# h3jia/bayesfast

Hardware: AMD Instinct MI355X
Metric: leapfrog steps/sec (all chains), 4096 chains x 64-d quadratic surrogate (higher is better)
Workload: dtype f64

## Files before the change

### bayesfast_amd/csrc/bfhip_api.hip

```cpp
#include <cmath>
#include <cstdarg>
#include <cstdio>
#include <cstdlib>
#include <cstring>
#include <vector>
#include "bfhip_common.h"
#include "bfhip_pack.h"

static thread_local char g_err[512] = "";

int bf_set_error(int code, const char *fmt, ...) {
    va_list ap;
    va_start(ap, fmt);
    vsnprintf(g_err, sizeof(g_err), fmt, ap);
    va_end(ap);
    return code;
}

static int env_int(const char *name, int dflt) { const char *e = getenv(name); return e ? atoi(e) : dflt; }
BfTune &bf_tune() {
    static BfTune t = [] {
        BfTune u;
        memset(&u, 0, sizeof(u));
        const char *nk = getenv("BFHIP_NUTS_KERNEL");
        u.no_group = env_int("BFHIP_NO_GROUP", (nk && (!strcmp(nk, "sliced") || !strcmp(nk, "pipe"))) ? 1 : 0);
        u.no_pipe = env_int("BFHIP_NO_PIPE", (nk && !strcmp(nk, "sliced")) ? 1 : 0);
        u.no_plain = env_int("BFHIP_NO_PLAIN", 0);
        u.no_quad = env_int("BFHIP_NO_QUAD", 0);
        u.wave_cpg = env_int("BFHIP_WAVE_CPG", 0);
        u.tail_relaunch = env_int("BFHIP_TAIL_RELAUNCH", 1);
        u.tail_stop = env_int("BFHIP_TAIL_STOP", 4);
        u.tail_q = env_int("BFHIP_TAIL_Q", 3);
        u.tail_max = env_int("BFHIP_TAIL_MAX", 4);
        u.lone = env_int("BFHIP_LONE", 1);
        u.lone_form = env_int("BFHIP_LONE_FORM", -1);
        u.pld_waves = env_int("BFHIP_PLD_WAVES", 0);
        u.cubic_form = env_int("BFHIP_CUBIC_FORM", 0);
        u.cubic_loops = env_int("BFHIP_CUBIC_LOOPS", 0);
        u.gram_one_wave = env_int("BFHIP_GRAM_ONE_WAVE", 0);
        u.chol_one_panel = env_int("BFHIP_CHOL_ONE_PANEL", 0);
        u.no_vel_ahead = env_int("BFHIP_NO_VEL_AHEAD", 0);
        u.tnuts_wpb = env_int("BFHIP_TNUTS_WPB", 0);
        u.tnuts_generic = env_int("BFHIP_TNUTS_GENERIC", 0);
        u.no_bound_proof = env_int("BFHIP_NO_BOUND_PROOF", 0);
        u.no_proof_weights = env_int("BFHIP_NO_PROOF_WEIGHTS", 0);
        u.pld_no_compress = env_int("BFHIP_PLD_NO_COMPRESS", 0);
        u.pld_stream = env_int("BFHIP_PLD_STREAM", 0);
        u.pld_no_cl = env_int("BFHIP_PLD_NO_CL", 0);
        u.no_decay_shared = env_int("BFHIP_NO_DECAY_SHARED", 0);
        u.polar_tiles = env_int("BFHIP_POLAR_TILES", 0);
        u.no_group_pld = env_int("BFHIP_NO_GROUP_PLD", 0);
        return u;
    }();
    return t;
}
static int *tune_field(const char *key) {
    BfTune &t = bf_tune();
    struct { const char *k; int *p; } tab[] = {
        {"no_group", &t.no_group}, {"no_pipe", &t.no_pipe}, {"no_plain", &t.no_plain}, {"no_quad", &t.no_quad}, {"wave_cpg", &t.wave_cpg},
        {"tail_relaunch", &t.tail_relaunch}, {"tail_stop", &t.tail_stop}, {"tail_q", &t.tail_q}, {"tail_max", &t.tail_max}, {"lone", &t.lone}, {"lone_form", &t.lone_form},
        {"pld_waves", &t.pld_waves}, {"cubic_form", &t.cubic_form}, {"cubic_loops", &t.cubic_loops}, {"gram_one_wave", &t.gram_one_wave}, {"chol_one_panel", &t.chol_one_panel}, {"no_vel_ahead", &t.no_vel_ahead}, {"tnuts_wpb", &t.tnuts_wpb}, {"tnuts_generic", &t.tnuts_generic}, {"no_bound_proof", &t.no_bound_proof},
        {"no_proof_weights", &t.no_proof_weights}, {"pld_no_compress", &t.pld_no_compress}, {"pld_stream", &t.pld_stream}, {"pld_no_cl", &t.pld_no_cl}, {"no_decay_shared", &t.no_decay_shared}, {"polar_tiles", &t.polar_tiles}, {"no_group_pld", &t.no_group_pld}};
    for (auto &e : tab)
        if (key && !strcmp(key, e.k)) return e.p;
    return NULL;
}
extern "C" int bfhip_debug_set(const char *key, long long value) {
    int *f = tune_field(key);
    if (!f) return bf_set_error(BFHIP_ERR_ARG, "bfhip_debug_set: unknown switch '%s'", key ? key : "(null)");
    *f = (int)value;
    return 0;
}
extern "C" long long bfhip_debug_get(const char *key) {
    const int *f = tune_field(key);
    return f ? *f : 0;
}
extern "C" int bfhip_debug_buffer(const char *key, void *device_ptr) {
    BfTune &t = bf_tune();
    unsigned long long *p = (unsigned long long *)device_ptr;
    if (key && !strcmp(key, "stamps")) t.stamps = p;
    else if (key && !strcmp(key, "stamps_lone")) t.stamps_lone = p;
    else if (key && !strcmp(key, "gstamps")) t.gstamps = p;
    else if (key && !strcmp(key, "group_counters")) t.group_counters = p;
    else return bf_set_error(BFHIP_ERR_ARG, "bfhip_debug_buffer: unknown buffer '%s'", key ? key : "(null)");
    return 0;
}
extern "C" const char *bfhip_debug_last_kernel(void) { return bf_tune().last_kernel; }

extern "C" int bfhip_version(void) { return 108; }
extern "C" const char *bfhip_last_error(void) { return g_err; }

extern "C" int bfhip_ctx_create(bfhip_ctx **out, int device, void *stream) {
    if (!out) return bf_set_error(BFHIP_ERR_ARG, "bfhip_ctx_create: out is NULL");
    int n_dev = 0;
    BF_HIP_CHECK(hipGetDeviceCount(&n_dev));
    if (device < 0 || device >= n_dev) return bf_set_error(BFHIP_ERR_ARG, "bfhip_ctx_create: device %d of %d", device, n_dev);
    BF_HIP_CHECK(hipSetDevice(device));
    hipDeviceProp_t prop;
    BF_HIP_CHECK(hipGetDeviceProperties(&prop, device));
    if (strncmp(prop.gcnArchName, "gfx950", 6) != 0)
        return bf_set_error(BFHIP_ERR_UNSUPPORTED, "bfhip is built for gfx950 only, found %s", prop.gcnArchName);
    bfhip_ctx *c = (bfhip_ctx *)calloc(1, sizeof(bfhip_ctx));
    c->device = device;
    c->stream = (hipStream_t)stream;
    c->n_cu = prop.multiProcessorCount;
    *out = c;
    return 0;
}

extern "C" void bfhip_ctx_destroy(bfhip_ctx *ctx) {
    if (!ctx) return;
    if (ctx->model_buf) (void)hipFree(ctx->model_buf);
    if (ctx->scratch) (void)hipFree(ctx->scratch);
    if (ctx->cubic_buf) (void)hipFree(ctx->cubic_buf);
    if (ctx->pm_buf) (void)hipFree(ctx->pm_buf);
    if (ctx->pld_buf) (void)hipFree(ctx->pld_buf);
    if (ctx->tail_buf) (void)hipFree(ctx->tail_buf);
    if (ctx->flow) (void)hipFree(ctx->flow);
    if (ctx->hess_work) (void)hipFree(ctx->hess_work);
    free(ctx);
}

extern "C" int bfhip_ctx_set_stream(bfhip_ctx *ctx, void *stream) {
    if (!ctx) return bf_set_error(BFHIP_ERR_ARG, "ctx is NULL");
    ctx->stream = (hipStream_t)stream;
    return 0;
}

extern "C" int bfhip_ctx_synchronize(bfhip_ctx *ctx) {
    if (!ctx) return bf_set_error(BFHIP_ERR_ARG, "ctx is NULL");
    BF_HIP_CHECK(hipStreamSynchronize(ctx->stream));
    return 0;
}

extern "C" int bfhip_density_upload(bfhip_ctx *ctx, const bfhip_density_desc *ds) {
    BfDeviceGuard dev_guard(ctx);
    if (!ctx || !ds) return bf_set_error(BFHIP_ERR_ARG, "bfhip_density_upload: NULL argument");
    const int d = ds->d;
    if (d < 1 || d > BFHIP_MAX_DIM) return bf_set_error(BFHIP_ERR_ARG, "bfhip_density_upload: d = %d out of [1, %d]", d, BFHIP_MAX_DIM);
    if (ds->use_bound && (!ds->mu || !ds->hess || !(ds->alpha > 0.)))
        return bf_set_error(BFHIP_ERR_ARG, "use_bound needs mu, hess and alpha > 0");
    if (ds->use_decay && (!ds->decay_mu || !ds->decay_hess))
        return bf_set_error(BFHIP_ERR_ARG, "use_decay needs decay_mu and decay_hess");
    if ((ds->su_lo == NULL) != (ds->su_diff == NULL)) return bf_set_error(BFHIP_ERR_ARG, "su_lo and su_diff go together");
    std::vector<double> h;
    const int DP = bf_pack_density(ds, h);
    const size_t MAT = (size_t)DP * DP, n_dbl = h.size();
    BF_HIP_CHECK(hipSetDevice(ctx->device));
    const size_t bytes = n_dbl * sizeof(double);
    if (int rc = bf_grow(ctx, &ctx->model_buf, &ctx->model_bytes, bytes)) return rc;
    BF_HIP_CHECK(hipStreamSynchronize(ctx->stream));
    BF_HIP_CHECK(hipMemcpy(ctx->model_buf, h.data(), bytes, hipMemcpyHostToDevice));
    DevModel &m = ctx->model;
    memset(&m, 0, sizeof(m));
    m.d = d;
    m.DP = DP;
    m.has_transform = ds->ranges != NULL;
    m.has_su = ds->su_lo != NULL;
    m.has_quad = ds->quad != NULL;
    m.use_bound = ds->use_bound != 0;
    m.use_decay = ds->use_decay != 0;
    m.decay_shared = ds->use_bound && ds->use_decay && memcmp(ds->decay_hess, ds->hess, (size_t)d * d * sizeof(double)) == 0 &&
                     memcmp(ds->decay_mu, ds->mu, (size_t)d * sizeof(double)) == 0;
    const double *base = (const double *)ctx->model_buf;
    m.pd = base;
    m.Sf = base + (size_t)PD_N * DP;
    m.Hf = m.Sf + MAT;
    m.Hdf = m.Hf + MAT;
    if (m.decay_shared) m.Hdf = m.Hf;
    m.c0 = ds->c0;
    m.alpha = ds->alpha;
    m.lam_max = ds->use_bound ? bf_bound_lam_max_weighted(ds->hess, ds->d, h.data() + (size_t)PD_HD * DP) : 0.;
    m.lam_max_d = ds->use_decay ? bf_bound_lam_max_weighted(ds->decay_hess, ds->d, h.data() + (size_t)PD_HDD * DP) : 0.;
    m.f_mu = ds->f_mu;
// ... 128 lines not shown
```

### bayesfast_amd/csrc/bfhip_common.h

```cpp
#pragma once
#include <hip/hip_runtime.h>
#include <stdint.h>
#include "../../include/bfhip.h"
#include "bfhip_model.h"
#include "bfhip_tune.h"

__device__ inline double bf_shfl_xor(double v, int mask) { return __shfl_xor(v, mask, 64); }

__device__ inline double bf_logaddexp(double x, double y) {
    if (x == y) return x + 0.6931471805599453094;
    double tmp = x - y;
    if (tmp > 0) return x + log1p(exp(-tmp));
    if (tmp <= 0) return y + log1p(exp(tmp));
    return tmp;
}

__device__ inline uint64_t bf_order_key(double v) {
    if (v != v) return ~0ull;
    if (v == 0.) v = 0.;
    const uint64_t b = (uint64_t)__double_as_longlong(v);
    return (b >> 63) ? ~b : (b | 0x8000000000000000ull);
}

#define BF_HIP_CHECK(expr)                                                                 \
// ... 13 lines not shown
    size_t model_bytes;
    void *cubic_buf;
    size_t cubic_bytes;
    void *pm_buf;
    size_t pm_bytes;
    int has_pm;
    void *pld_buf;
    size_t pld_bytes;
    struct PolyDev {
        int d, DP, m, use_bound, has_quad;
        const double *Sf;
        const double *lin;
        const double *c0;
        const double *f_mu;
        const double *mu;
        const double *Hf;
        double alpha;
        int n2, n3;
        const int *mask2, *pos2, *mask3, *pos3;
        const double *A2, *A2t, *T3t;
    } pm;
    int *tail_buf;
    size_t tail_bytes;
    void *scratch;
    size_t scratch_bytes;
    int n_cu;
    void *flow;
    size_t flow_bytes;
    void *hess_work;
    size_t hess_work_bytes;
};

struct BfDeviceGuard {
    int prev = -1;
    explicit BfDeviceGuard(const bfhip_ctx *ctx) {
        if (ctx && hipGetDevice(&prev) == hipSuccess && prev != ctx->device) (void)hipSetDevice(ctx->device);
        else prev = -1;
    }
    ~BfDeviceGuard() { if (prev >= 0) (void)hipSetDevice(prev); }
};

#define BF_LDS_MAX ((size_t)160 * 1024)

template <typename K>
static inline int bf_set_lds(K kern, size_t bytes) {
    if (bytes > 64 * 1024)
// ... 23 lines not shown
```

### bayesfast_amd/csrc/bfhip_lone.h

```cpp

#pragma push_macro("exp")
#pragma push_macro("log")
#pragma push_macro("sqrt")
#pragma push_macro("sincospi")
#undef exp
#undef log
#undef sqrt
#undef sincospi
__device__ inline double ln_opq(double x) { asm("" : "+v"(x)); return x; }
#define LN_EXPV(x) ln_opq(exp(ln_opq(x)))
#define LN_LOGV(x) ln_opq(log(ln_opq(x)))
#define LN_SQRTV(x) ln_opq(sqrt(ln_opq(x)))
#define LN_EXP(x) rfl(LN_EXPV(x))
#define LN_LOG(x) rfl(LN_LOGV(x))
#define LN_SQRT(x) rfl(LN_SQRTV(x))

enum { LN_CONT = 0, LN_NEW = 1, LN_DONE = 2 };
enum { LF_NONE = 0, LF_LEAF = 1, LF_INIT = 2 };
enum { LV_CMD = 0, LV_CLOSE, LV_EO, LV_EVAL, LV_DIR, LV_INIT, LV_N = 8 };

template <int W, int DEC>
struct LoneGeo {
    using PG = PipeGeo<W, DEC>;
    static constexpr int DP = 16 * W, NS = 4 * W, NMAT = PG::NMAT, KS = PG::KS, KPJ = PG::KPJ;
// ... 711 lines not shown
                    dir_use = bf_pipe_dir(bf_xoshiro_next(t));
                }
            }
            if (lane == 0) {
                VI[LV_CMD] = LN_CONT; VI[LV_CLOSE] = close; VI[LV_EO] = eo; VI[LV_EVAL] = ev; VI[LV_DIR] = dir_use;
            }
            fly = ev ? LF_LEAF : LF_NONE;
        }
        LTRACE(1, 3);
#ifdef BF_LTRACE
        ltrip += 1;
#endif
    }
#undef KBAR

#ifdef BF_LTRACE
    if (a.stamps && blockIdx.x == 0)
        for (int i = lane; i < BF_LTRACE * 32; i += 64) a.stamps[i] = LTRC[i];
#endif
    if (err == 2 && lane_ok) q = LF[lane];
    store_vec(BFHIP_VEC_Q, q);
    if (lane == 0) {
        for (int k = 0; k < 4; ++k) a.rng[(size_t)chain * 4 + k] = rs[k];
        scp[BFHIP_SC_LOG_STEP] = log_step;
        scp[BFHIP_SC_LOG_BAR] = log_bar;
        scp[BFHIP_SC_HBAR] = hbar;
        scp[BFHIP_SC_COUNT] = count;
        scp[BFHIP_SC_I_ITER] = (double)i_iter;
        scp[BFHIP_SC_ERROR] = (double)err;
        if (a.n_leapfrog && nlf) atomicAdd(a.n_leapfrog, nlf);
    }
}
#undef LN_EXP
#undef LN_LOG
#undef LN_SQRT
#undef LN_EXPV
#undef LN_LOGV
#undef LN_SQRTV
#pragma pop_macro("exp")
#pragma pop_macro("log")
#pragma pop_macro("sqrt")
#pragma pop_macro("sincospi")
```

### bayesfast_amd/csrc/bfhip_nuts_pipe.h

```cpp


enum { SL_PROPG = SL_STACK + 4 * BFHIP_MAX_TREEDEPTH, SL_PG = SL_PROPG + 1, SL_PIPE_N = SL_PG + BFHIP_MAX_TREEDEPTH };

template <int W, int DEC = 0>
struct PipeGeo {
    static constexpr int NMAT = DEC == 1 ? 3 : 2;
    static constexpr int KS = DEC == 1 ? (W == 2 ? 2 : 1) : ((W == 2 || W == 4) ? 2 : 1);
    static constexpr int KPJ = (4 * W) / KS, NJOB = NMAT * W * KS, NTL = 12;
    static constexpr int MPS = KPJ > 8 ? 2 : 1;
    static_assert(NJOB <= 16 && KPJ <= 8 * MPS, "one job per wave, eight MFMA sites");
    static constexpr size_t lds_doubles() {
        using G = SamplerGeo<W>;
        return (size_t)NMAT * G::NS * G::XS + (size_t)16 * BFHIP_MAX_TREEDEPTH * LS_N + 4 + (size_t)16 * CS_N +
               (size_t)16 * NTL * G::DP + (size_t)NMAT * KS * 16 * G::GS;
    }
};

template <int QUAD> struct PipeAcc { typedef d4_t type; };
template <> struct PipeAcc<1> { typedef double type; };
template <> struct PipeAcc<2> { typedef d2_t type; };
__device__ inline d4_t bf_pipe_mfma(double a_, double b_, d4_t c_) { return __builtin_amdgcn_mfma_f64_16x16x4f64(a_, b_, c_, 0, 0, 0); }
__device__ inline double bf_pipe_mfma(double a_, double b_, double c_) { return __builtin_amdgcn_mfma_f64_4x4x4f64(a_, b_, c_, 0, 0, 0); }

__device__ inline double bf_pipe_u01(uint64_t x) {
// ... 12 lines not shown
    constexpr int DP = G::DP, NS = G::NS, XS = G::XS, GS = G::GS;
    constexpr int KS_P = PG::KS, KPJ_P = PG::KPJ, NJOB_P = PG::NJOB, NTL = PG::NTL, NMAT = PG::NMAT, MPS = PG::MPS;
    constexpr int MAXL = BFHIP_MAX_TREEDEPTH;
    static_assert(DP <= 64, "one dimension per lane");
    extern __shared__ __attribute__((aligned(16))) double lds[];
    double *XB = lds;
    double *LS = XB + NMAT * NS * XS;
    int *alive = (int *)(LS + 16 * MAXL * LS_N);
    double *CS = LS + 16 * MAXL * LS_N + 4;
    double *TB = CS + 16 * CS_N;
    double *GB = TB + 16 * NTL * DP;

    const int tid = threadIdx.x, lane = tid & 63;
    const int w = __builtin_amdgcn_readfirstlane(tid >> 6);
    int cpg = a.cpg > 0 ? a.cpg : 16;
    int chain = blockIdx.x * cpg + w;
    bool real = w < cpg && chain < a.n_chain;
    if (a.tail_list) {
        const int cnt = rfl(a.tail_count[0]);
        cpg = cnt <= a.n_cu ? 1 : (cnt <= 2 * a.n_cu ? 2 : 4);
        const int idx = blockIdx.x * cpg + w;
        real = w < cpg && idx < cnt;
        chain = real ? rfl(a.tail_list[idx]) : 0;
    }
    const int d = m.d;
    const bool lane_ok = lane < DP;

    double afr[KPJ_P];
    {
        const int slot_m = w / (W * KS_P), rem = w % (W * KS_P), t = rem / KS_P, kp = rem % KS_P;
        const double *Af = (slot_m == 0 ? m.Sf : (slot_m == 1 ? m.Hf : m.Hdf)) + (t * NS + kp * KPJ_P) * 64 + lane;
#pragma unroll
        for (int s = 0; s < KPJ_P; ++s) afr[s] = (w < NJOB_P) ? Af[s * 64] : 0.;
    }
    if (tid < 8) alive[tid] = 0;
    const double c_lin = lane_ok ? m.pd[PD_LIN * DP + lane] : 0.;
    const double c_mu = lane_ok ? m.pd[PD_MU * DP + lane] : 0.;
    const double c_dmu = (DEC == 1 && lane_ok) ? m.pd[PD_DMU * DP + lane] : 0.;
    const double c_smu = lane_ok ? m.pd[PD_SMU * DP + lane] : 0.;
    const int c_kind = (TR && lane_ok) ? (int)m.pd[PD_KIND * DP + lane] : 0;
    const double c_lo = (TR && lane_ok) ? m.pd[PD_LO * DP + lane] : 0., c_rg = (TR && lane_ok) ? m.pd[PD_RG * DP + lane] : 1.;
    double xs = 0., jac = 1., gj = 0., logdet_l = 0.;

    double q = 0., p = 0., g = 0., var = 1.;
    double TLp = 0., TPs = 0., TPq = 0.;
    double TRp = 0.;
// ... 44 lines not shown
        double sn, cs;
        sincospi(2. * u2, &sn, &cs);
        const double z = (lane & 1) ? rad * sn : rad * cs;
        p = (lane < d) ? (1. / sqrt(var)) * z : 0.;
        g = 0.;
    };
    if (real) {
        for (int k = 0; k < 4; ++k) rs[k] = rfl((uint64_t)a.rng[(size_t)chain * 4 + k]);
        cs_set(CS_LOG_STEP, rfl(scp[BFHIP_SC_LOG_STEP]));
        cs_set(CS_LOG_BAR, rfl(scp[BFHIP_SC_LOG_BAR]));
        cs_set(CS_HBAR, rfl(scp[BFHIP_SC_HBAR]));
        cs_set(CS_SMU, rfl(scp[BFHIP_SC_MU]));
        cs_set(CS_COUNT, rfl(scp[BFHIP_SC_COUNT]));
        cs_set(CS_STEP_NOW, uexp(rfl(scp[BFHIP_SC_LOG_STEP])));
        cs_set(CS_STEP_BAR, uexp(rfl(scp[BFHIP_SC_LOG_BAR])));
        i_iter = rfl((int)scp[BFHIP_SC_I_ITER]);
        err = rfl((int)scp[BFHIP_SC_ERROR]);
        q = load_vec(BFHIP_VEC_Q, 0.);
        var = load_vec(BFHIP_VEC_VAR, 1.);
        if (i_iter < a.iter_end && err == 0) {
            mode = M_INIT;
            draw_momentum();
        } else if (a.tail_done && lane == 0) {
            atomicAdd(a.tail_done, 1);
        }
    }
    __syncthreads();
    if (lane == 0 && mode == M_DONE) atomicAdd(&alive[6], 1);

#ifdef BF_TRACE
    __shared__ unsigned long long TRC[BF_TRACE * 16];
    for (int i = threadIdx.x; i < BF_TRACE * 16; i += 1024) TRC[i] = 0;
    int trip_no = 0;
#endif
    auto init_tree = [&](double E0, double logp0) {
        if (!(fabs(E0) <= 1.7976931348623157e308)) {
            err = 1;
        } else {
            start_energy = E0;
            stv(SL_LEFT_Q, q); stv(SL_LEFT_P, p); stv(SL_LEFT_G, g);
            stv(SL_RIGHT_Q, q); stv(SL_RIGHT_P, p); stv(SL_RIGHT_G, g);
            stv(SL_PROP_Q, q); stv(SL_PSUM, p);
            stv(SL_PROPG, g);
            cs_set(CS_PROP_E, E0);
            cs_set(CS_PROP_LOGP, logp0);
            cs_set(CS_TREE_W, 1.);
            w_off = 0.;
// ... 73 lines not shown
                    prev_upd = n_samples;
                    if (a.cfg.doubling) adapt_window *= 2.;
                }
                n_samples += 1.;
                store_vec(BFHIP_VEC_FG_MEAN, fm);
                store_vec(BFHIP_VEC_FG_RAW, fr);
                store_vec(BFHIP_VEC_BG_MEAN, bm);
                store_vec(BFHIP_VEC_BG_RAW, br);
                if (lane == 0) {
                    scp[BFHIP_SC_FG_N] = fg_n;
                    scp[BFHIP_SC_BG_N] = bg_n;
                    scp[BFHIP_SC_N_SAMPLES] = n_samples;
                    scp[BFHIP_SC_PREV_UPDATE] = prev_upd;
                    scp[BFHIP_SC_ADAPT_WINDOW] = adapt_window;
                }
            }
            i_iter += 1;
            TRACE(12);
            bool go_on = i_iter < a.iter_end && err == 0;
            if (go_on && a.tail_stop > 0 && a.iter_end - i_iter >= 8) {
                const int i_iter0 = rfl((int)scp[BFHIP_SC_I_ITER]);
                if (4 * (a.iter_end - i_iter) >= a.iter_end - i_iter0 && 16 - rfl(alive[6]) <= a.tail_stop) {
                    const int dg = rfl(__hip_atomic_load(a.tail_done, __ATOMIC_RELAXED, __HIP_MEMORY_SCOPE_AGENT));
                    if (4 * dg >= a.tail_q * a.n_chain) go_on = false;
                }
            }
            if (go_on) {
                mode = M_INIT;
                draw_momentum();
            } else {
                mode = M_DONE;
                if (lane == 0) {
                    atomicAdd(&alive[6], 1);
                    if (a.tail_done && (i_iter >= a.iter_end || err != 0)) atomicAdd(a.tail_done, 1);
                }
            }
        }
    };

    auto gb_read = [&](int slot_m) -> double {
        const double *gp = GB + ((slot_m * KS_P) * 16 + w) * GS + lane;
        double r = gp[0];
        if (KS_P > 1) r += gp[16 * GS];
        return r;
    };

    for (int trip = 0;; ++trip) {
#ifdef BF_TRACE
        trip_no = trip;
#endif
        TRACE(0);
        bool evaluating = false, turn = false;
        int eo2 = 0;
        if (mode == M_INIT) {
            evaluating = true;
        } else if (mode == M_LEAF) {
            evaluating = true;
// ... 383 lines not shown
                } else if constexpr (DEC == 2) {
                    r_a[0] = pc.get(2); r_a[1] = pc.get(3);
                } else {
                    r_a[0] = xm * gmu; r_a[1] = xm * sv;
                    wave_sum_n<2>(r_a);
                }
                const BfOob o = bf_oob_scalars(m.alpha, m.inv_alpha, m.f_mu, m.f_poly_mu, beta, r_a[0], r_a[1]);
                f = o.f;
                gn = bf_oob_grad(o, gmu, sv, hv);
                kin_ready = false;
            }
            finish(f, gn, kin_ready, r_kin, logdet, r_bd2, dgr);
        }
    }

#ifdef BF_TRACE
    if (a.stamps && w == 0 && blockIdx.x == 0)
        for (int i = lane; i < BF_TRACE * 16; i += 64) a.stamps[i] = TRC[i];
#endif
    if (real) {
        store_vec(BFHIP_VEC_Q, q);
        if (lane == 0) {
            for (int k = 0; k < 4; ++k) a.rng[(size_t)chain * 4 + k] = rs[k];
            scp[BFHIP_SC_LOG_STEP] = cs_get(CS_LOG_STEP);
            scp[BFHIP_SC_LOG_BAR] = cs_get(CS_LOG_BAR);
            scp[BFHIP_SC_HBAR] = cs_get(CS_HBAR);
            scp[BFHIP_SC_COUNT] = cs_get(CS_COUNT);
            scp[BFHIP_SC_I_ITER] = (double)i_iter;
            scp[BFHIP_SC_ERROR] = (double)err;
            if (a.n_leapfrog && nlf) atomicAdd(a.n_leapfrog, nlf);
        }
    }
}
```

### bayesfast_amd/csrc/bfhip_sampler.hip

```cpp
#include <type_traits>
#include <cstring>
#include <cstdio>
#include <cstdlib>
#include "bfhip_eval.h"
#include "bfhip_metric.h"
#include "bfhip_pld.h"
#include "bfhip_oob.h"

__device__ __attribute__((noinline)) static double bf_exp_ni(double x) { return exp(x); }
__device__ __attribute__((noinline)) static double bf_log_ni(double x) { return log(x); }
__device__ __attribute__((noinline)) static double bf_sqrt_ni(double x) { return sqrt(x); }
__device__ __attribute__((noinline)) static void bf_sincospi_ni(double x, double *s, double *c) { sincospi(x, s, c); }
#define exp(x) bf_exp_ni(x)
#define log(x) bf_log_ni(x)
#define sqrt(x) bf_sqrt_ni(x)
#define sincospi(x, s, c) bf_sincospi_ni(x, s, c)
#define uexp(x) rfl(bf_exp_ni(x))
#define ulog(x) rfl(bf_log_ni(x))
#define usqrt(x) rfl(bf_sqrt_ni(x))

#include "bfhip_sampler_defs.h"

#include "bfhip_wave.h"

// ... 1637 lines not shown
    args.cub_lds = sampler_cubic_lds(ctx->model, FS == 1) ? 1 : 0;
    args.cub_loops = tune.cubic_loops;
    const int groups = (args.n_chain + args.cpg - 1) / args.cpg;
    snprintf(tune.last_kernel, sizeof(tune.last_kernel), "bf_sampler_kernel<%d, %s, %s, %d, %d>", W, NUTS ? "true" : "false",
             STAMPS ? "true" : "false", FS, FULLM);
    hipLaunchKernelGGL(k, dim3(groups), dim3(NWV * 64), lds, ctx->stream, ctx->model, args);
    BF_HIP_CHECK(hipGetLastError());
    return 0;
}

extern "C" int bfhip_debug_tail_count(bfhip_ctx *ctx) {
    if (!ctx || !ctx->tail_buf) return -1;
    int n = -1;
    if (hipStreamSynchronize(ctx->stream) != hipSuccess) return -1;
    if (hipMemcpy(&n, ctx->tail_buf, sizeof(int), hipMemcpyDeviceToHost) != hipSuccess) return -1;
    return n;
}
static int tail_stop_now() {
    const BfTune &tune = bf_tune();
    const int hi = tune.lone ? 16 : 4;
    return tune.tail_stop < 1 ? 1 : (tune.tail_stop > hi ? hi : tune.tail_stop);
}

__global__ void bf_tail_list_kernel(int n_chain, int iter_end, const double *sc, int *buf) {
    const int i = blockIdx.x * blockDim.x + threadIdx.x;
    if (i >= n_chain) return;
    const double *scp = sc + (size_t)i * BFHIP_SC_N;
    if ((int)scp[BFHIP_SC_I_ITER] < iter_end && (int)scp[BFHIP_SC_ERROR] == 0) buf[2 + atomicAdd(buf, 1)] = i;
}




template <int W> struct LoneOcc { static constexpr int MINW = W == 1 ? 2 : 3; };

using SamplerKernel = void (*)(DevModel, SamplerArgs);
template <int W, bool TR, int DEC, int FORM>
static SamplerKernel lone_kernel() {
    if constexpr (FORM == 0) return bf_lone_kernel<W, TR, DEC, 1, 0>;
    else if constexpr (FORM == 1) return bf_lone_kernel<W, TR, DEC, 1, (W == 4 ? 1 : 0)>;
    else return bf_lone_kernel<W, TR, DEC, LoneOcc<W>::MINW, 0>;
}
template <int W, int DEC, int FORM> constexpr int lone_threads() { return LoneWaves<W, DEC, (FORM == 1 && W == 4) ? 1 : 0>::NW * 64; }

template <int W, bool TR, int DEC, int FORM>
static int lone_blocks_per_cu(bfhip_ctx *ctx) {
    static int cached[64];
    static bool have[64];
    const int dev = (ctx->device >= 0 && ctx->device < 64) ? ctx->device : 0;
    if (have[dev]) return cached[dev];
    const size_t lds = LoneGeo<W, DEC>::n_doubles * sizeof(double);
    const SamplerKernel k = lone_kernel<W, TR, DEC, FORM>();
    int nb = 0;
    if (bf_set_lds(k, lds) != 0) return 0;
    if (hipOccupancyMaxActiveBlocksPerMultiprocessor(&nb, k, lone_threads<W, DEC, FORM>(), lds) != hipSuccess) return 0;
    cached[dev] = nb;
    have[dev] = true;
    return nb;
}

template <int W, bool TR, int DEC, int FORM>
static int lone_launch_form(bfhip_ctx *ctx, const SamplerArgs &args, int n_blocks) {
    const size_t lds = LoneGeo<W, DEC>::n_doubles * sizeof(double);
    const SamplerKernel k = lone_kernel<W, TR, DEC, FORM>();
    if (int rc = bf_set_lds(k, lds)) return rc;
    hipLaunchKernelGGL(k, dim3(n_blocks), dim3(lone_threads<W, DEC, FORM>()), lds, ctx->stream, ctx->model, args);
    BF_HIP_CHECK(hipGetLastError());
    return 0;
}

template <int W, bool TR, int DEC>
static int launch_lone(bfhip_ctx *ctx, const SamplerArgs &args_in, int n_blocks, bool tail) {
    BfTune &tune = bf_tune();
    if (!tune.lone || args_in.stamps) return 0;
    SamplerArgs args = args_in;
    args.n_cu = ctx->n_cu;
    args.tail_stop = 0;
    args.tail_done = NULL;
    if (!tail) { args.tail_list = NULL; args.tail_count = NULL; }
    args.stamps = tune.stamps_lone;
    const int need = (n_blocks + ctx->n_cu - 1) / ctx->n_cu;
    int form = 0;
    if (lone_blocks_per_cu<W, TR, DEC, 0>(ctx) < need) {
        form = 1;
        if (W != 4 || lone_blocks_per_cu<W, TR, DEC, 1>(ctx) < need) {
            form = 2;
            if (tune.lone != 2 && !tail) return 0;
        }
    }
    if (tune.lone_form >= 0 && tune.lone_form <= 2) form = tune.lone_form;
    const int rc = form == 0 ? lone_launch_form<W, TR, DEC, 0>(ctx, args, n_blocks)
                 : form == 1 ? lone_launch_form<W, TR, DEC, 1>(ctx, args, n_blocks) : lone_launch_form<W, TR, DEC, 2>(ctx, args, n_blocks);
    if (rc) return rc;
    if (!tail) snprintf(tune.last_kernel, sizeof(tune.last_kernel), "bf_lone_kernel<%d, %s, %d, %d>", W, TR ? "true" : "false", DEC, form);
    return 1;
}

template <int W, bool TR = false, int DEC = 0>
static int launch_nuts_pipe(bfhip_ctx *ctx, const SamplerArgs &args_in) {
    BfTune &tune = bf_tune();
    SamplerArgs args = args_in;
    args.cpg = wave_layout_cpg(ctx, args.n_chain, 16);
    args.tail_stop = 0;
    args.tail_list = NULL;
    args.tail_count = NULL;
    args.tail_done = NULL;
    args.n_cu = ctx->n_cu;
    const int quad = tune.no_quad ? 0 : (args.cpg <= 4 ? 1 : (args.cpg <= 8 ? 2 : 0));
    auto k = quad == 1 ? bf_nuts_pipe_kernel<W, TR, DEC, 1> : (quad == 2 ? bf_nuts_pipe_kernel<W, TR, DEC, 2> : bf_nuts_pipe_kernel<W, TR, DEC, 0>);
    if ((quad == 1 && tune.wave_cpg == 0) || tune.lone == 2) {
        const int r = launch_lone<W, TR, DEC>(ctx, args, args.n_chain, false);
        if (r != 0) return r < 0 ? r : 0;
    }
    const size_t lds = PipeGeo<W, DEC>::lds_doubles() * sizeof(double);
    if (int rc = bf_set_lds(k, lds)) return rc;
    const int groups = (args.n_chain + args.cpg - 1) / args.cpg;
    const bool two_parts = tune.tail_relaunch && args.cpg == 16 && !tune.no_quad && !args.stamps;
    if (two_parts) {
        if (int rc = bf_grow(ctx, (void **)&ctx->tail_buf, &ctx->tail_bytes, (size_t)(args.n_chain + 2) * sizeof(int))) return rc;
        args.tail_stop = tail_stop_now();
        args.tail_q = tune.tail_q < 1 ? 1 : (tune.tail_q > 4 ? 4 : tune.tail_q);
        args.tail_done = ctx->tail_buf + 1;
        BF_HIP_CHECK(hipMemsetAsync(ctx->tail_buf, 0, 2 * sizeof(int), ctx->stream));
    }
    hipLaunchKernelGGL(k, dim3(groups), dim3(1024), lds, ctx->stream, ctx->model, args);
    BF_HIP_CHECK(hipGetLastError());
    snprintf(tune.last_kernel, sizeof(tune.last_kernel), "bf_nuts_pipe_kernel<%d, %s, %d, %d>", W, TR ? "true" : "false", DEC, quad);
    if (two_parts) {
        hipLaunchKernelGGL(bf_tail_list_kernel, dim3((args.n_chain + 255) / 256), dim3(256), 0, ctx->stream, args.n_chain, args.iter_end, args.sc,
                           ctx->tail_buf);
        BF_HIP_CHECK(hipGetLastError());
        auto k2 = bf_nuts_pipe_kernel<W, TR, DEC, 1>;
        if (int rc = bf_set_lds(k2, lds)) return rc;
        SamplerArgs a2 = args;
        a2.tail_stop = 0;
        a2.tail_count = ctx->tail_buf;
        a2.tail_list = ctx->tail_buf + 2;
        a2.tail_done = NULL;
        a2.cpg = 4;
        {
            const int most = args.n_chain < args.tail_stop * groups ? args.n_chain : args.tail_stop * groups;
            const int r = launch_lone<W, TR, DEC>(ctx, a2, most, true);
            if (r != 0) return r < 0 ? r : 0;
        }
        const int groups2 = groups > ctx->n_cu ? groups : ctx->n_cu;
        hipLaunchKernelGGL(k2, dim3(groups2), dim3(1024), lds, ctx->stream, ctx->model, a2);
        BF_HIP_CHECK(hipGetLastError());
    }
    return 0;
}

template <int W, bool NUTS>
static int launch_sampler(bfhip_ctx *ctx, const SamplerArgs &args) {
    const BfTune &tune = bf_tune();
    const DevModel &m = ctx->model;
    const bool plain = sampler_plain(m) && !args.mat;
    if (m.pld.on && m.pld.stream) {
        if (sampler_lds_bytes(m, false, 8) > BF_LDS_MAX)
            return bf_set_error(BFHIP_ERR_UNSUPPORTED, "bfhip_sampler_run: this streamed pipeline density needs %zu KB of LDS at d = %d (160 KB)",
                                sampler_lds_bytes(m, false, 8) / 1024, m.d);
        return args.mat ? launch_sampler_t<W, NUTS, false, 11, 1>(ctx, args) : launch_sampler_t<W, NUTS, false, 11>(ctx, args);
    }
    if (m.pld.on) {
        if constexpr (W == 8) {
            if (sampler_lds_bytes(m, false, 8) > BF_LDS_MAX)
                return bf_set_error(BFHIP_ERR_UNSUPPORTED, "bfhip_sampler_run: this pipeline density needs %zu KB of LDS at d = %d (160 KB)",
                                    sampler_lds_bytes(m, false, 8) / 1024, m.d);
            return args.mat ? launch_sampler_t<8, NUTS, false, 9, 1>(ctx, args) : launch_sampler_t<8, NUTS, false, 9>(ctx, args);
        } else {
            if (args.mat) {
                return launch_sampler_t<W, NUTS, false, 9, 1>(ctx, args);
            }
// ... 70 lines not shown
        return bf_set_error(BFHIP_ERR_ARG, "invalid sampler configuration");
    const DevModel &m = ctx->model;
    const int W = m.DP / 16;
    SamplerArgs args;
    args.cpg = 0;
    args.cub_lds = 0;
    args.no_quad = tune.no_quad;
    args.cfg = *cfg;
    args.n_chain = n_chain;
    args.iter_end = iter_end;
    args.iter_out0 = iter_out0;
    args.n_out = n_out;
    args.nslot = SL_PIPE_N;
    args.tail_max = tune.tail_max;
    args.ks = sampler_ksplit(m);
    args.gbn = sampler_gb_slots(m);
    args.rng = rng;
    args.sc = sc;
    args.vec = vec;
    args.samples = samples;
    args.stats = stats;
    args.n_leapfrog = n_leapfrog;
    args.stamps = tune.stamps;
    args.no_bound_proof = bf_no_bound_proof();
    args.gcount = NULL;
    args.mat = (cfg->full_metric && cfg->metric_mat) ? cfg->metric_mat : NULL;
    if (cfg->full_metric && !cfg->metric_mat) return bf_set_error(BFHIP_ERR_ARG, "bfhip_sampler_run: full_metric without metric_mat");
    const size_t need = (size_t)((n_chain + 15) / 16 * 16) * args.nslot * m.DP * sizeof(double);
    if (int rc = bf_grow(ctx, &ctx->scratch, &ctx->scratch_bytes, need)) return rc;
    args.scratch = (double *)ctx->scratch;
    const bool nuts = cfg->sampler == 0;
    if (cfg->chain_layout < 0 || cfg->chain_layout > 3) return bf_set_error(BFHIP_ERR_ARG, "chain_layout should be 0, 1, 2 or 3");
    const bool lanes = !tune.no_group && !tune.no_pipe && !tune.no_plain && !args.stamps;
    if (cfg->chain_layout == 3 && lanes && bf_split_supports(m, args)) return bf_launch_split(ctx, args);
    const bool want_group = cfg->chain_layout == 1 || cfg->chain_layout == 3 || (cfg->chain_layout == 0 && !nuts);
    if (want_group && lanes && bf_group_supports(m, args)) return bf_launch_group(ctx, args);
    switch (W) {
#ifndef BF_ONLY_HEADLINE
    case 1: return nuts ? launch_sampler<1, true>(ctx, args) : launch_sampler<1, false>(ctx, args);
    case 2: return nuts ? launch_sampler<2, true>(ctx, args) : launch_sampler<2, false>(ctx, args);
    case 8: return nuts ? launch_sampler<8, true>(ctx, args) : launch_sampler<8, false>(ctx, args);
#endif
    case 4: return nuts ? launch_sampler<4, true>(ctx, args) : launch_sampler<4, false>(ctx, args);
    }
    return bf_set_error(BFHIP_ERR_UNSUPPORTED, "unsupported padded dimension %d", m.DP);
}
// ... 124 lines not shown
```

### bayesfast_amd/csrc/bfhip_sampler_defs.h

```cpp
#pragma once
#include "bfhip_model.h"

struct SamplerArgs {
    bfhip_sampler_config cfg;
    int n_chain, iter_end, iter_out0, n_out, nslot;
    int cpg;
    int no_quad;
    int cub_lds;
    int pld_cl;
    int tail_max;
    int ks, gbn;
    uint64_t *rng;
    double *sc, *vec, *samples, *stats;
    unsigned long long *n_leapfrog;
    double *scratch;
    double *mat;
    unsigned long long *gcount;
    int no_bound_proof;
    int tail_stop, n_cu;
    int tail_q;
    int cub_loops;
    const int *tail_list, *tail_count;
    int *tail_done;
    unsigned long long *stamps;
};

enum { M_INIT = 0, M_LEAF = 1, M_OOB = 2, M_DONE = 3 };
enum { U_EVAL = 0, U_MERGE_RUN, U_DBL_END, U_END1, U_END2, U_END3, U_DONE, U_MERGE, U_ABORT };
enum { SL_LEFT_Q = 0, SL_LEFT_P, SL_LEFT_G, SL_RIGHT_Q, SL_RIGHT_P, SL_RIGHT_G, SL_PROP_Q, SL_PSUM, SL_STACK };
enum { LS_LS = 0, LS_E, LS_LOGP, LS_ACC, LS_N };
enum { CS_LOG_STEP = 0, CS_LOG_BAR, CS_HBAR, CS_SMU, CS_COUNT, CS_PROP_E, CS_PROP_LOGP, CS_MAX_DE, CS_HACC, CS_HDE,
       CS_W_OFF, CS_TREE_W, CS_BETA, CS_T_E, CS_T_LOGP, CS_STEP_NOW, CS_STEP_BAR, CS_N };


size_t bf_sampler_lds_bytes_base(const DevModel &m);
int bf_pld_logp_grad(struct bfhip_ctx *ctx, int n, const double *x, int original_space, double *logp, double *grad);
struct bfhip_ctx;
bool bf_group_supports(const DevModel &m, const SamplerArgs &args);
int bf_launch_group(bfhip_ctx *ctx, const SamplerArgs &args);
int bf_no_bound_proof();
bool bf_split_supports(const DevModel &m, const SamplerArgs &args);
int bf_launch_split(bfhip_ctx *ctx, const SamplerArgs &args);
```

### bayesfast_amd/csrc/bfhip_tune.h

```cpp
#pragma once

struct BfTune {
    int no_group;
    int no_pipe;
    int no_plain;
    int no_quad;
    int wave_cpg;
    int tail_relaunch;
    int tail_stop;
    int tail_q;
    int tail_max;
    int lone;
    int lone_form;
    int pld_waves;
    int cubic_form;
    int gram_one_wave;
    int chol_one_panel;
    int cubic_loops;
    int no_vel_ahead;
    int tnuts_wpb;
    int tnuts_generic;
    int no_bound_proof;
    int no_proof_weights;
    int no_group_pld;
    int polar_tiles;
    int no_decay_shared;
    int pld_no_cl;
    int pld_no_compress;
    int pld_stream;
    unsigned long long *stamps, *stamps_lone, *gstamps, *group_counters;
    char last_kernel[96];
};

BfTune &bf_tune();
```

Measured before the change: 793.8 million.

## Launch historically slowest chains early on a side stream alongside the pipe kernel

```diff
diff --git a/bayesfast_amd/csrc/bfhip_api.hip b/bayesfast_amd/csrc/bfhip_api.hip
--- a/bayesfast_amd/csrc/bfhip_api.hip
+++ b/bayesfast_amd/csrc/bfhip_api.hip
@@ -34,6 +34,7 @@
         u.tail_max = env_int("BFHIP_TAIL_MAX", 4);
         u.lone = env_int("BFHIP_LONE", 1);
         u.lone_form = env_int("BFHIP_LONE_FORM", -1);
+        u.early_max = env_int("BFHIP_EARLY_MAX", -1);
         u.pld_waves = env_int("BFHIP_PLD_WAVES", 0);
         u.cubic_form = env_int("BFHIP_CUBIC_FORM", 0);
         u.cubic_loops = env_int("BFHIP_CUBIC_LOOPS", 0);
@@ -58,7 +59,7 @@
     BfTune &t = bf_tune();
     struct { const char *k; int *p; } tab[] = {
         {"no_group", &t.no_group}, {"no_pipe", &t.no_pipe}, {"no_plain", &t.no_plain}, {"no_quad", &t.no_quad}, {"wave_cpg", &t.wave_cpg},
-        {"tail_relaunch", &t.tail_relaunch}, {"tail_stop", &t.tail_stop}, {"tail_q", &t.tail_q}, {"tail_max", &t.tail_max}, {"lone", &t.lone}, {"lone_form", &t.lone_form},
+        {"tail_relaunch", &t.tail_relaunch}, {"tail_stop", &t.tail_stop}, {"tail_q", &t.tail_q}, {"tail_max", &t.tail_max}, {"lone", &t.lone}, {"lone_form", &t.lone_form}, {"early_max", &t.early_max},
         {"pld_waves", &t.pld_waves}, {"cubic_form", &t.cubic_form}, {"cubic_loops", &t.cubic_loops}, {"gram_one_wave", &t.gram_one_wave}, {"chol_one_panel", &t.chol_one_panel}, {"no_vel_ahead", &t.no_vel_ahead}, {"tnuts_wpb", &t.tnuts_wpb}, {"tnuts_generic", &t.tnuts_generic}, {"no_bound_proof", &t.no_bound_proof},
         {"no_proof_weights", &t.no_proof_weights}, {"pld_no_compress", &t.pld_no_compress}, {"pld_stream", &t.pld_stream}, {"pld_no_cl", &t.pld_no_cl}, {"no_decay_shared", &t.no_decay_shared}, {"polar_tiles", &t.polar_tiles}, {"no_group_pld", &t.no_group_pld}};
     for (auto &e : tab)
@@ -82,12 +83,14 @@
     else if (key && !strcmp(key, "stamps_lone")) t.stamps_lone = p;
     else if (key && !strcmp(key, "gstamps")) t.gstamps = p;
     else if (key && !strcmp(key, "group_counters")) t.group_counters = p;
+    else if (key && !strcmp(key, "early_list")) t.early_list = (int *)device_ptr;
+    else if (key && !strcmp(key, "work_record")) t.work_record = (int *)device_ptr;
     else return bf_set_error(BFHIP_ERR_ARG, "bfhip_debug_buffer: unknown buffer '%s'", key ? key : "(null)");
     return 0;
 }
 extern "C" const char *bfhip_debug_last_kernel(void) { return bf_tune().last_kernel; }
 
-extern "C" int bfhip_version(void) { return 108; }
+extern "C" int bfhip_version(void) { return 109; }
 extern "C" const char *bfhip_last_error(void) { return g_err; }
 
 extern "C" int bfhip_ctx_create(bfhip_ctx **out, int device, void *stream) {
@@ -116,6 +119,10 @@
     if (ctx->pm_buf) (void)hipFree(ctx->pm_buf);
     if (ctx->pld_buf) (void)hipFree(ctx->pld_buf);
     if (ctx->tail_buf) (void)hipFree(ctx->tail_buf);
+    if (ctx->early_buf) (void)hipFree(ctx->early_buf);
+    if (ctx->ev_main) (void)hipEventDestroy(ctx->ev_main);
+    if (ctx->ev_side) (void)hipEventDestroy(ctx->ev_side);
+    if (ctx->side_stream) (void)hipStreamDestroy(ctx->side_stream);
     if (ctx->flow) (void)hipFree(ctx->flow);
     if (ctx->hess_work) (void)hipFree(ctx->hess_work);
     free(ctx);
@@ -150,6 +157,7 @@
     const size_t bytes = n_dbl * sizeof(double);
     if (int rc = bf_grow(ctx, &ctx->model_buf, &ctx->model_bytes, bytes)) return rc;
     BF_HIP_CHECK(hipStreamSynchronize(ctx->stream));
+    ctx->early.valid = 0;
     BF_HIP_CHECK(hipMemcpy(ctx->model_buf, h.data(), bytes, hipMemcpyHostToDevice));
     DevModel &m = ctx->model;
     memset(&m, 0, sizeof(m));
diff --git a/bayesfast_amd/csrc/bfhip_common.h b/bayesfast_amd/csrc/bfhip_common.h
--- a/bayesfast_amd/csrc/bfhip_common.h
+++ b/bayesfast_amd/csrc/bfhip_common.h
@@ -59,6 +59,13 @@
     } pm;
     int *tail_buf;
     size_t tail_bytes;
+    int *early_buf;
+    size_t early_bytes;
+    int early_n, early_dirty;
+    struct { const void *sc, *vec; int n_chain, iter_end, iter_out0, cap, valid; unsigned seq; } early;
+    unsigned run_seq;
+    hipStream_t side_stream;
+    hipEvent_t ev_main, ev_side;
     void *scratch;
     size_t scratch_bytes;
     int n_cu;
diff --git a/bayesfast_amd/csrc/bfhip_lone.h b/bayesfast_amd/csrc/bfhip_lone.h
--- a/bayesfast_amd/csrc/bfhip_lone.h
+++ b/bayesfast_amd/csrc/bfhip_lone.h
@@ -757,6 +757,11 @@
     store_vec(BFHIP_VEC_Q, q);
     if (lane == 0) {
         for (int k = 0; k < 4; ++k) a.rng[(size_t)chain * 4 + k] = rs[k];
+        {
+            int *wk = BF_WORK_OF(a, chain);
+            wk[0] += (int)nlf;
+            wk[1] += i_iter - (int)scp[BFHIP_SC_I_ITER];
+        }
         scp[BFHIP_SC_LOG_STEP] = log_step;
         scp[BFHIP_SC_LOG_BAR] = log_bar;
         scp[BFHIP_SC_HBAR] = hbar;
diff --git a/bayesfast_amd/csrc/bfhip_nuts_pipe.h b/bayesfast_amd/csrc/bfhip_nuts_pipe.h
--- a/bayesfast_amd/csrc/bfhip_nuts_pipe.h
+++ b/bayesfast_amd/csrc/bfhip_nuts_pipe.h
@@ -58,6 +58,8 @@
         const int idx = blockIdx.x * cpg + w;
         real = w < cpg && idx < cnt;
         chain = real ? rfl(a.tail_list[idx]) : 0;
+    } else if (real) {
+        real = rfl(*BF_EARLY_FLAG_OF(a, chain)) == 0;
     }
     const int d = m.d;
     const bool lane_ok = lane < DP;
@@ -148,7 +150,7 @@
             mode = M_INIT;
             draw_momentum();
         } else if (a.tail_done && lane == 0) {
-            atomicAdd(a.tail_done, 1);
+            atomicAdd(a.tail_done, 4);
         }
     }
     __syncthreads();
@@ -268,7 +270,7 @@
                 const int i_iter0 = rfl((int)scp[BFHIP_SC_I_ITER]);
                 if (4 * (a.iter_end - i_iter) >= a.iter_end - i_iter0 && 16 - rfl(alive[6]) <= a.tail_stop) {
                     const int dg = rfl(__hip_atomic_load(a.tail_done, __ATOMIC_RELAXED, __HIP_MEMORY_SCOPE_AGENT));
-                    if (4 * dg >= a.tail_q * a.n_chain) go_on = false;
+                    if (dg >= a.tail_q * a.n_chain) go_on = false;
                 }
             }
             if (go_on) {
@@ -278,7 +280,7 @@
                 mode = M_DONE;
                 if (lane == 0) {
                     atomicAdd(&alive[6], 1);
-                    if (a.tail_done && (i_iter >= a.iter_end || err != 0)) atomicAdd(a.tail_done, 1);
+                    if (a.tail_done && (i_iter >= a.iter_end || err != 0)) atomicAdd(a.tail_done, 4);
                 }
             }
         }
@@ -708,6 +710,11 @@
         store_vec(BFHIP_VEC_Q, q);
         if (lane == 0) {
             for (int k = 0; k < 4; ++k) a.rng[(size_t)chain * 4 + k] = rs[k];
+            {
+                int *wk = BF_WORK_OF(a, chain);
+                wk[0] += (int)nlf;
+                wk[1] += i_iter - (int)scp[BFHIP_SC_I_ITER];
+            }
             scp[BFHIP_SC_LOG_STEP] = cs_get(CS_LOG_STEP);
             scp[BFHIP_SC_LOG_BAR] = cs_get(CS_LOG_BAR);
             scp[BFHIP_SC_HBAR] = cs_get(CS_HBAR);
diff --git a/bayesfast_amd/csrc/bfhip_sampler.hip b/bayesfast_amd/csrc/bfhip_sampler.hip
--- a/bayesfast_amd/csrc/bfhip_sampler.hip
+++ b/bayesfast_amd/csrc/bfhip_sampler.hip
@@ -1683,13 +1683,74 @@
     return tune.tail_stop < 1 ? 1 : (tune.tail_stop > hi ? hi : tune.tail_stop);
 }
 
-__global__ void bf_tail_list_kernel(int n_chain, int iter_end, const double *sc, int *buf) {
+__global__ void bf_tail_list_kernel(int n_chain, int iter_end, const double *sc, int *buf, const int *early_flag) {
     const int i = blockIdx.x * blockDim.x + threadIdx.x;
     if (i >= n_chain) return;
+    if (early_flag && early_flag[i]) return;
     const double *scp = sc + (size_t)i * BFHIP_SC_N;
     if ((int)scp[BFHIP_SC_I_ITER] < iter_end && (int)scp[BFHIP_SC_ERROR] == 0) buf[2 + atomicAdd(buf, 1)] = i;
 }
 
+
+#define BF_EARLY_CAP 1024
+__global__ __launch_bounds__(1024) void bf_early_list_kernel(int n_chain, int early_max, const int *work, int *buf, int *flag,
+                                                             unsigned long long *total, unsigned long long *user_total) {
+    __shared__ unsigned long long red[1024];
+    __shared__ unsigned long long tot[1024];
+    const int tid = threadIdx.x;
+    unsigned long long mx = 0, sum = 0;
+    for (int c = tid; c < n_chain; c += 1024) {
+        const unsigned long long w_ = (unsigned long long)(unsigned)work[2 * c];
+        mx = w_ > mx ? w_ : mx;
+        sum += w_;
+        flag[c] = 0;
+    }
+    red[tid] = mx; tot[tid] = sum;
+    __syncthreads();
+    for (int s_ = 512; s_ > 0; s_ >>= 1) {
+        if (tid < s_) { red[tid] = red[tid + s_] > red[tid] ? red[tid + s_] : red[tid]; tot[tid] += tot[tid + s_]; }
+        __syncthreads();
+    }
+    mx = red[0]; sum = tot[0];
+    __syncthreads();
+    unsigned long long last = ~0ull;
+    int n = 0;
+    for (; n < early_max && n < BF_EARLY_CAP; ++n) {
+        unsigned long long best = 0;
+        for (int c = tid; c < n_chain; c += 1024) {
+            const unsigned long long w_ = (unsigned long long)(unsigned)work[2 * c];
+            if (w_ == 0 || 2 * w_ < mx || w_ * (unsigned long long)n_chain < 4 * sum) continue;
+            const unsigned long long key = (w_ << 32) | (unsigned long long)(0xffffffffu - (unsigned)c);
+            if (key < last && key > best) best = key;
+        }
+        red[tid] = best;
+        __syncthreads();
+        for (int s_ = 512; s_ > 0; s_ >>= 1) {
+            if (tid < s_) red[tid] = red[tid + s_] > red[tid] ? red[tid + s_] : red[tid];
+            __syncthreads();
+        }
+        best = red[0];
+        __syncthreads();
+        if (best == 0) break;
+        last = best;
+        if (tid == 0) {
+            const int c = (int)(0xffffffffu - (unsigned)(best & 0xffffffffull));
+            buf[1 + n] = c;
+            flag[c] = 1;
+        }
+    }
+    if (tid == 0) {
+        buf[0] = n;
+        if (user_total && *total) atomicAdd(user_total, *total);
+        *total = 0;
+    }
+}
+static int early_max_now(const bfhip_ctx *ctx) {
+    const BfTune &tune = bf_tune();
+    int e = tune.early_max < 0 ? ctx->n_cu / 16 : tune.early_max;
+    if (e > ctx->n_cu) e = ctx->n_cu;
+    return e > BF_EARLY_CAP ? BF_EARLY_CAP : e;
+}
 
 
 
@@ -1721,11 +1782,11 @@
 }
 
 template <int W, bool TR, int DEC, int FORM>
-static int lone_launch_form(bfhip_ctx *ctx, const SamplerArgs &args, int n_blocks) {
+static int lone_launch_form(bfhip_ctx *ctx, const SamplerArgs &args, int n_blocks, hipStream_t stream) {
     const size_t lds = LoneGeo<W, DEC>::n_doubles * sizeof(double);
     const SamplerKernel k = lone_kernel<W, TR, DEC, FORM>();
     if (int rc = bf_set_lds(k, lds)) return rc;
-    hipLaunchKernelGGL(k, dim3(n_blocks), dim3(lone_threads<W, DEC, FORM>()), lds, ctx->stream, ctx->model, args);
+    hipLaunchKernelGGL(k, dim3(n_blocks), dim3(lone_threads<W, DEC, FORM>()), lds, stream, ctx->model, args);
     BF_HIP_CHECK(hipGetLastError());
     return 0;
 }
@@ -1750,11 +1811,103 @@
         }
     }
     if (tune.lone_form >= 0 && tune.lone_form <= 2) form = tune.lone_form;
-    const int rc = form == 0 ? lone_launch_form<W, TR, DEC, 0>(ctx, args, n_blocks)
-                 : form == 1 ? lone_launch_form<W, TR, DEC, 1>(ctx, args, n_blocks) : lone_launch_form<W, TR, DEC, 2>(ctx, args, n_blocks);
+    const int rc = form == 0 ? lone_launch_form<W, TR, DEC, 0>(ctx, args, n_blocks, ctx->stream)
+                 : form == 1 ? lone_launch_form<W, TR, DEC, 1>(ctx, args, n_blocks, ctx->stream)
+                             : lone_launch_form<W, TR, DEC, 2>(ctx, args, n_blocks, ctx->stream);
     if (rc) return rc;
     if (!tail) snprintf(tune.last_kernel, sizeof(tune.last_kernel), "bf_lone_kernel<%d, %s, %d, %d>", W, TR ? "true" : "false", DEC, form);
     return 1;
+}
+
+struct EarlyLane {
+    int *count, *list, *flag, *work;
+    unsigned long long *total, *user_total;
+    bool use;
+    int cap;
+};
+__global__ void bf_count_flush_kernel(unsigned long long *total, unsigned long long *user_total) {
+    if (user_total && *total) atomicAdd(user_total, *total);
+    *total = 0;
+}
+__global__ void bf_tail_open_kernel(int *buf, const int *early_count, int tail_q) {
+    buf[0] = 0;
+    buf[1] = early_count ? tail_q * early_count[0] : 0;
+}
+static int early_lane_open(bfhip_ctx *ctx, SamplerArgs &args, EarlyLane &e, bool two_parts) {
+    const BfTune &tune = bf_tune();
+    const size_t head = 1 + BF_EARLY_CAP + 1;
+    const size_t need = (head + 2 + 3 * (size_t)args.n_chain) * sizeof(int);
+    const auto was = ctx->early;
+    ctx->early.valid = 0;
+    if (int rc = bf_grow(ctx, (void **)&ctx->early_buf, &ctx->early_bytes, need)) return rc;
+    const bool fresh = ctx->early_n != args.n_chain;
+    if (fresh) {
+        BF_HIP_CHECK(hipMemsetAsync(ctx->early_buf, 0, need, ctx->stream));
+        ctx->early_n = args.n_chain;
+        ctx->early_dirty = 0;
+    }
+    e.count = ctx->early_buf;
+    e.list = e.count + 1;
+    e.total = (unsigned long long *)(ctx->early_buf + head);
+    e.work = (int *)(e.total + 1);
+    e.flag = e.work + 2 * (size_t)args.n_chain;
+    e.user_total = args.n_leapfrog;
+    args.n_leapfrog = e.total;
+    e.cap = early_max_now(ctx);
+    e.use = two_parts && !fresh && was.valid && was.seq + 1 == ctx->run_seq && was.sc == (const void *)args.sc &&
+            was.vec == (const void *)args.vec && was.n_chain == args.n_chain && args.iter_end > was.iter_end &&
+            (args.iter_out0 == was.iter_out0 || args.iter_out0 == was.iter_end) && tune.lone && e.cap > 0 && was.cap == e.cap;
+    if (!e.use && ctx->early_dirty) {
+        BF_HIP_CHECK(hipMemsetAsync(e.flag, 0, (size_t)args.n_chain * sizeof(int), ctx->stream));
+        ctx->early_dirty = 0;
+    }
+    if (two_parts) BF_HIP_CHECK(hipMemsetAsync(e.work, 0, 2 * (size_t)args.n_chain * sizeof(int), ctx->stream));
+    return 0;
+}
+template <int W, bool TR, int DEC>
+static int early_lane_start(bfhip_ctx *ctx, const SamplerArgs &args, const EarlyLane &e) {
+    if (!ctx->side_stream) {
+        BF_HIP_CHECK(hipStreamCreateWithFlags(&ctx->side_stream, hipStreamNonBlocking));
+        BF_HIP_CHECK(hipEventCreateWithFlags(&ctx->ev_main, hipEventDisableTiming));
+        BF_HIP_CHECK(hipEventCreateWithFlags(&ctx->ev_side, hipEventDisableTiming));
+    }
+    BF_HIP_CHECK(hipEventRecord(ctx->ev_main, ctx->stream));
+    BF_HIP_CHECK(hipStreamWaitEvent(ctx->side_stream, ctx->ev_main, 0));
+    SamplerArgs ae = args;
+    ae.tail_stop = 0;
+    ae.tail_done = NULL;
+    ae.tail_count = e.count;
+    ae.tail_list = e.list;
+    ae.stamps = NULL;
+    if (int rc = lone_launch_form<W, TR, DEC, 0>(ctx, ae, e.cap, ctx->side_stream)) return rc;
+    BF_HIP_CHECK(hipEventRecord(ctx->ev_side, ctx->side_stream));
+    return 0;
+}
+static int early_lane_close(bfhip_ctx *ctx, const SamplerArgs &args, const EarlyLane &e, bool two_parts) {
+    const BfTune &tune = bf_tune();
+    if (!two_parts) {
+        hipLaunchKernelGGL(bf_count_flush_kernel, dim3(1), dim3(1), 0, ctx->stream, e.total, e.user_total);
+        BF_HIP_CHECK(hipGetLastError());
+        return 0;
+    }
+    if (e.use) BF_HIP_CHECK(hipStreamWaitEvent(ctx->stream, ctx->ev_side, 0));
+    hipLaunchKernelGGL(bf_early_list_kernel, dim3(1), dim3(1024), 0, ctx->stream, args.n_chain, e.cap, e.work, e.count, e.flag, e.total,
+                       e.user_total);
+    BF_HIP_CHECK(hipGetLastError());
+    if (tune.early_list)
+        BF_HIP_CHECK(hipMemcpyAsync(tune.early_list, e.count, (1 + BF_EARLY_CAP) * sizeof(int), hipMemcpyDeviceToDevice, ctx->stream));
+    if (tune.work_record)
+        BF_HIP_CHECK(hipMemcpyAsync(tune.work_record, e.work, 2 * (size_t)args.n_chain * sizeof(int), hipMemcpyDeviceToDevice, ctx->stream));
+    ctx->early_dirty = e.cap > 0;
+    ctx->early.sc = args.sc;
+    ctx->early.vec = args.vec;
+    ctx->early.n_chain = args.n_chain;
+    ctx->early.iter_end = args.iter_end;
+    ctx->early.iter_out0 = args.iter_out0;
+    ctx->early.cap = e.cap;
+    ctx->early.seq = ctx->run_seq;
+    ctx->early.valid = 1;
+    return 0;
 }
 
 template <int W, bool TR = false, int DEC = 0>
@@ -1769,27 +1922,38 @@
     args.n_cu = ctx->n_cu;
     const int quad = tune.no_quad ? 0 : (args.cpg <= 4 ? 1 : (args.cpg <= 8 ? 2 : 0));
     auto k = quad == 1 ? bf_nuts_pipe_kernel<W, TR, DEC, 1> : (quad == 2 ? bf_nuts_pipe_kernel<W, TR, DEC, 2> : bf_nuts_pipe_kernel<W, TR, DEC, 0>);
-    if ((quad == 1 && tune.wave_cpg == 0) || tune.lone == 2) {
+    const bool whole_lone = ((quad == 1 && tune.wave_cpg == 0) || tune.lone == 2) && tune.lone && !args.stamps;
+    const bool two_parts = tune.tail_relaunch && args.cpg == 16 && !tune.no_quad && !args.stamps;
+    EarlyLane early;
+    if (int rc = early_lane_open(ctx, args, early, two_parts && !whole_lone)) return rc;
+    if (whole_lone) {
         const int r = launch_lone<W, TR, DEC>(ctx, args, args.n_chain, false);
-        if (r != 0) return r < 0 ? r : 0;
+        if (r < 0) return r;
+        if (r != 0) return early_lane_close(ctx, args, early, false);
     }
     const size_t lds = PipeGeo<W, DEC>::lds_doubles() * sizeof(double);
     if (int rc = bf_set_lds(k, lds)) return rc;
     const int groups = (args.n_chain + args.cpg - 1) / args.cpg;
-    const bool two_parts = tune.tail_relaunch && args.cpg == 16 && !tune.no_quad && !args.stamps;
+    const int *early_flag = NULL;
     if (two_parts) {
         if (int rc = bf_grow(ctx, (void **)&ctx->tail_buf, &ctx->tail_bytes, (size_t)(args.n_chain + 2) * sizeof(int))) return rc;
         args.tail_stop = tail_stop_now();
         args.tail_q = tune.tail_q < 1 ? 1 : (tune.tail_q > 4 ? 4 : tune.tail_q);
         args.tail_done = ctx->tail_buf + 1;
-        BF_HIP_CHECK(hipMemsetAsync(ctx->tail_buf, 0, 2 * sizeof(int), ctx->stream));
+        hipLaunchKernelGGL(bf_tail_open_kernel, dim3(1), dim3(1), 0, ctx->stream, ctx->tail_buf, early.use ? early.count : (const int *)NULL,
+                           args.tail_q);
+        BF_HIP_CHECK(hipGetLastError());
+        if (early.use) {
+            if (int rc = early_lane_start<W, TR, DEC>(ctx, args, early)) return rc;
+            early_flag = early.flag;
+        }
     }
     hipLaunchKernelGGL(k, dim3(groups), dim3(1024), lds, ctx->stream, ctx->model, args);
     BF_HIP_CHECK(hipGetLastError());
     snprintf(tune.last_kernel, sizeof(tune.last_kernel), "bf_nuts_pipe_kernel<%d, %s, %d, %d>", W, TR ? "true" : "false", DEC, quad);
     if (two_parts) {
         hipLaunchKernelGGL(bf_tail_list_kernel, dim3((args.n_chain + 255) / 256), dim3(256), 0, ctx->stream, args.n_chain, args.iter_end, args.sc,
-                           ctx->tail_buf);
+                           ctx->tail_buf, early_flag);
         BF_HIP_CHECK(hipGetLastError());
         auto k2 = bf_nuts_pipe_kernel<W, TR, DEC, 1>;
         if (int rc = bf_set_lds(k2, lds)) return rc;
@@ -1799,16 +1963,16 @@
         a2.tail_list = ctx->tail_buf + 2;
         a2.tail_done = NULL;
         a2.cpg = 4;
-        {
-            const int most = args.n_chain < args.tail_stop * groups ? args.n_chain : args.tail_stop * groups;
-            const int r = launch_lone<W, TR, DEC>(ctx, a2, most, true);
-            if (r != 0) return r < 0 ? r : 0;
-        }
-        const int groups2 = groups > ctx->n_cu ? groups : ctx->n_cu;
-        hipLaunchKernelGGL(k2, dim3(groups2), dim3(1024), lds, ctx->stream, ctx->model, a2);
-        BF_HIP_CHECK(hipGetLastError());
-    }
-    return 0;
+        const int most = args.n_chain < args.tail_stop * groups ? args.n_chain : args.tail_stop * groups;
+        const int r = launch_lone<W, TR, DEC>(ctx, a2, most, true);
+        if (r < 0) return r;
+        if (r == 0) {
+            const int groups2 = groups > ctx->n_cu ? groups : ctx->n_cu;
+            hipLaunchKernelGGL(k2, dim3(groups2), dim3(1024), lds, ctx->stream, ctx->model, a2);
+            BF_HIP_CHECK(hipGetLastError());
+        }
+    }
+    return early_lane_close(ctx, args, early, two_parts);
 }
 
 template <int W, bool NUTS>
@@ -1925,6 +2089,7 @@
     args.stats = stats;
     args.n_leapfrog = n_leapfrog;
     args.stamps = tune.stamps;
+    ctx->run_seq += 1;
     args.no_bound_proof = bf_no_bound_proof();
     args.gcount = NULL;
     args.mat = (cfg->full_metric && cfg->metric_mat) ? cfg->metric_mat : NULL;
diff --git a/bayesfast_amd/csrc/bfhip_sampler_defs.h b/bayesfast_amd/csrc/bfhip_sampler_defs.h
--- a/bayesfast_amd/csrc/bfhip_sampler_defs.h
+++ b/bayesfast_amd/csrc/bfhip_sampler_defs.h
@@ -25,6 +25,9 @@
     unsigned long long *stamps;
 };
 
+#define BF_WORK_OF(a, chain) ((int *)((a).n_leapfrog + 1) + 2 * (chain))
+#define BF_EARLY_FLAG_OF(a, chain) ((const int *)((a).n_leapfrog + 1) + 2 * (a).n_chain + (chain))
+
 enum { M_INIT = 0, M_LEAF = 1, M_OOB = 2, M_DONE = 3 };
 enum { U_EVAL = 0, U_MERGE_RUN, U_DBL_END, U_END1, U_END2, U_END3, U_DONE, U_MERGE, U_ABORT };
 enum { SL_LEFT_Q = 0, SL_LEFT_P, SL_LEFT_G, SL_RIGHT_Q, SL_RIGHT_P, SL_RIGHT_G, SL_PROP_Q, SL_PSUM, SL_STACK };
diff --git a/bayesfast_amd/csrc/bfhip_tune.h b/bayesfast_amd/csrc/bfhip_tune.h
--- a/bayesfast_amd/csrc/bfhip_tune.h
+++ b/bayesfast_amd/csrc/bfhip_tune.h
@@ -12,6 +12,7 @@
     int tail_max;
     int lone;
     int lone_form;
+    int early_max;
     int pld_waves;
     int cubic_form;
     int gram_one_wave;
@@ -29,6 +30,8 @@
     int pld_no_compress;
     int pld_stream;
     unsigned long long *stamps, *stamps_lone, *gstamps, *group_counters;
+    int *early_list;
+    int *work_record;
     char last_kernel[96];
 };
 
```

After: 804.2 million, median of 6. +1.3%, better.
